# facebookresearch/SlowFast

Measured on NVIDIA H100. Metric: clips/sec (fwd+bwd) SlowFast-8x8-R50, higher is better.
Workload: dtype bf16x3-split operands, f32 accumulate/storage

## Files before the change

include/slowfast_b200.h:

```cpp
#ifndef SLOWFAST_B200_H_
#define SLOWFAST_B200_H_

#include <stdint.h>

#ifdef __cplusplus
extern "C" {
#endif

const char* sfb_last_error(void);
int sfb_abi_version(void);
const char* sfb_build_arch(void);

typedef struct sfb_conv_desc {
  const void* a_hi;
  const void* a_lo;
  int32_t n, d, h, w, c;
  int64_t c_pitch;
  const void* b_hi;
  const void* b_lo;
  int32_t cout;
  int32_t kt, kh, kw;
  int32_t dil_t, dil_h, dil_w;
  int32_t str_t, str_h, str_w;
  int32_t low_t, low_h, low_w;
// ... 44 lines not shown

int sfb_set_wgrad_direct(int32_t enabled);

int sfb_zero_f32_2d(float* ptr, int64_t rows, int64_t c, int64_t pitch, void* stream);

int sfb_add_f32_2d(float* dst, const float* src, int64_t rows, int32_t c, int64_t dst_pitch, int64_t src_pitch,
                   void* stream);

int sfb_split_planes(const float* x, int64_t rows, int32_t c, int64_t x_pitch, void* hi, void* lo,
                     int64_t o_pitch, void* stream);
int sfb_input_pack(const float* x, int32_t n, int32_t c, int32_t t, int32_t h, int32_t w, int32_t c_pad, void* hi,
                   void* lo, void* stream);
int sfb_filter_pack(const float* w, int32_t cout, int32_t cin, int32_t taps_total, const int32_t* tapmap,
                    int32_t ntaps, int32_t transpose, int32_t cols_pad, void* hi, void* lo, void* stream);
int sfb_filter_unpack_grad(const float* dwm, float* dw, int32_t cout, int32_t cin, int32_t taps, int32_t cin_pad,
                           int32_t accumulate, void* stream);

int sfb_bn_finalize(const float* partials, int32_t m_tiles, int32_t c, int64_t count, const float* gamma,
                    const float* beta, float* running_mean, float* running_var, float momentum, float eps,
                    int32_t training, float* scale, float* shift, float* save_mean, float* save_invstd,
                    int32_t affine_c, void* stream);

int32_t sfb_bn_split_stats_tiles(int64_t rows, int64_t rows_per_clip, int32_t splits, int32_t c);
int sfb_bn_split_stats(const float* y, int64_t y_pitch, int64_t rows, int32_t c, int32_t splits, int64_t rows_per_clip,
                       float* partials, void* stream);

typedef struct sfb_bn_apply_desc {
  const float* y; int64_t y_pitch; const float* scale; const float* shift;
  const float* y2; int64_t y2_pitch; const float* scale2; const float* shift2;
  const void* res_hi; const void* res_lo; int64_t res_pitch;
  void* out_hi; void* out_lo; int64_t out_pitch;
  int64_t rows; int32_t c; int32_t relu;
  int32_t splits; int64_t rows_per_clip;
} sfb_bn_apply_desc;
int sfb_bn_apply(const sfb_bn_apply_desc* d, void* stream);

typedef struct sfb_bn_bwd_desc {
  const float* dout; int64_t dout_pitch;
  const void* mask_hi; int64_t mask_pitch;
  const float* y; int64_t y_pitch;
  const float* mean; const float* invstd; const float* gamma;
  float* dgamma; float* dbeta; int32_t accumulate_param_grads;
  int32_t training;
  void* dy_hi; void* dy_lo; int64_t dy_pitch;
  float* dres; int64_t dres_pitch; int32_t dres_accumulate;
  float* partials;
  float* coef;
  int64_t rows; int32_t c;
  int32_t c_valid;
  const float* mask_scale; const float* mask_shift;
  int32_t splits; int64_t rows_per_clip;
} sfb_bn_bwd_desc;
int32_t sfb_bn_bwd_blocks(int64_t rows, int32_t c, int32_t splits, int64_t rows_per_clip);
int sfb_bn_bwd(const sfb_bn_bwd_desc* d, void* stream);

typedef struct sfb_pool_desc {
  const float* y; const float* scale; const float* shift;
  int32_t n, t, h, w, c, oh, ow, kh, kw, sh, sw, ph, pw;
  void* out_hi; void* out_lo; int64_t out_pitch;
  uint8_t* argmax;
  const float* dout; int64_t dout_pitch;
  float* dz;
  int32_t splits;
} sfb_pool_desc;
int sfb_bn_relu_maxpool_fwd(const sfb_pool_desc* d, void* stream);
int sfb_bn_relu_maxpool_bwd(const sfb_pool_desc* d, void* stream);



typedef struct sfb_pool3d_desc {
  const void* in_hi; const void* in_lo; int64_t in_pitch;
  void* out_hi; void* out_lo; int64_t out_pitch;
  uint8_t* argmax;
  int32_t n, t, h, w, c, ot, oh, ow;
  int32_t kt, kh, kw, st, sh, sw, pt, ph, pw;
  const float* dout; int64_t dout_pitch;
  float* din; int64_t din_pitch; int32_t din_accumulate;
} sfb_pool3d_desc;
int sfb_maxpool3d_fwd(const sfb_pool3d_desc* d, void* stream);
int sfb_maxpool3d_bwd(const sfb_pool3d_desc* d, void* stream);

int sfb_stem_input_fold(const float* x, int32_t n, int32_t cin, int32_t t, int32_t h, int32_t w, void* hi, void* lo,
                        void* stream);
int sfb_stem_filter_fold(const float* w, float* dw, int32_t cout, int32_t cin, int32_t kt, int32_t kh, int32_t kw,
// ... 261 lines not shown
```

slowfast_b200/csrc/elementwise.cu:

```cuda
#include <cstdint>
#include <cstring>
#include <cuda_bf16.h>

#include "../../include/slowfast_b200.h"
#include "planes.cuh"
#include "runtime.h"

namespace sfb {

static int ew_sms() {
  int sms = kGridSms;
  device_limits(&sms, nullptr);
  return sms;
}
static int ew_grid(int64_t items, int block) { return capped_grid(items, block, int64_t(ew_sms()) * 8); }
static int rowlane_grid(int64_t rows, int cg, int block) {
  const int lanes_c = cg < block ? cg : block;
  const int lanes_r = block / lanes_c;
  return capped_grid(rows, lanes_r * 4, int64_t(ew_sms()) * 8);
}

struct f32x8 {
  float4 a, b;
};
// ... 172 lines not shown
    for (int k = 0; k < 8; ++k) {
      sm[threadIdx.x * 16 + k] = s1[k];
      sm[threadIdx.x * 16 + 8 + k] = s2[k];
    }
    __syncthreads();
    if (lr == 0 && g < cg) {
      for (int q = 1; q < lanes_r; ++q) {
#pragma unroll
        for (int k = 0; k < 8; ++k) {
          s1[k] += sm[(q * lanes_c + lc) * 16 + k];
          s2[k] += sm[(q * lanes_c + lc) * 16 + 8 + k];
        }
      }
#pragma unroll
      for (int k = 0; k < 8; ++k) {
        const int64_t ch = int64_t(s) * p.c + g * 8 + k;
        p.partials[ch * p.blocks_per_split + col] = s1[k];
        p.partials[sq + ch * p.blocks_per_split + col] = s2[k];
      }
    }
    __syncthreads();
  }
}

struct BnApplyParams {
  const float* y; int64_t y_pitch;
  const float* scale; const float* shift;
  const float* y2; int64_t y2_pitch;
  const float* scale2; const float* shift2;
  const __nv_bfloat16* r_hi; const __nv_bfloat16* r_lo; int64_t r_pitch;
  __nv_bfloat16* o_hi; __nv_bfloat16* o_lo; int64_t o_pitch;
  int64_t rows; int c; int relu;
  int splits; int64_t rows_per_clip;
};
__device__ __forceinline__ int split_of_row(int64_t r, int64_t rows_per_clip, int splits) {
  return int((r / rows_per_clip) % splits);
}
struct RowLanes {
  int lanes_c, lanes_r, lc, lr;
  __device__ __forceinline__ RowLanes(int cg) {
    lanes_c = cg < int(blockDim.x) ? cg : int(blockDim.x);
    lanes_r = blockDim.x / lanes_c;
    lc = threadIdx.x % lanes_c;
    lr = threadIdx.x / lanes_c;
  }
};
__global__ void __launch_bounds__(256) bn_apply_kernel(const BnApplyParams p) {
  const int cg = p.c / 8;
  const RowLanes L(cg);
  if (L.lr >= L.lanes_r) return;
  for (int g = L.lc; g < cg; g += L.lanes_c) {
    const int c = g * 8;
    float sc[8], sh[8], sc2[8], sh2[8];
    load8(p.scale + c, sc);
    load8(p.shift + c, sh);
    if (p.y2) {
      load8(p.scale2 + c, sc2);
      load8(p.shift2 + c, sh2);
    }
    int cur = 0;
    for (int64_t r = int64_t(blockIdx.x) * L.lanes_r + L.lr; r < p.rows; r += int64_t(gridDim.x) * L.lanes_r) {
      if (p.splits > 1) {
        const int s = split_of_row(r, p.rows_per_clip, p.splits);
        if (s != cur) {
          cur = s;
          const int64_t o = int64_t(s) * p.c + c;
          load8(p.scale + o, sc);
          load8(p.shift + o, sh);
          if (p.y2) {
            load8(p.scale2 + o, sc2);
            load8(p.shift2 + o, sh2);
          }
        }
      }
      float v[8];
      load8(p.y + r * p.y_pitch + c, v);
#pragma unroll
      for (int j = 0; j < 8; ++j) v[j] = fmaf(v[j], sc[j], sh[j]);
      if (p.y2) {
        float w[8];
        load8(p.y2 + r * p.y2_pitch + c, w);
#pragma unroll
        for (int j = 0; j < 8; ++j) v[j] += fmaf(w[j], sc2[j], sh2[j]);
      }
      if (p.r_hi) {
        float w[8];
        load_planes8(p.r_hi + r * p.r_pitch + c, p.r_lo ? p.r_lo + r * p.r_pitch + c : nullptr, w);
#pragma unroll
        for (int j = 0; j < 8; ++j) v[j] += w[j];
      }
      if (p.relu) {
#pragma unroll
        for (int j = 0; j < 8; ++j) v[j] = fmaxf(v[j], 0.f);
      }
      store_split8(p.o_hi + r * p.o_pitch + c, p.o_lo ? p.o_lo + r * p.o_pitch + c : nullptr, v);
    }
  }
}

struct BnBwdReduceParams {
  const float* dout; int64_t dout_pitch;
  const __nv_bfloat16* mask; int64_t mask_pitch;
  const float* y; int64_t y_pitch;
  const float* mean; const float* invstd;
  int64_t rows; int c;
  float* partials;
  const float* mask_scale; const float* mask_shift;
  int splits; int64_t rows_per_clip; int blocks_per_clip;
};
__global__ void __launch_bounds__(256) bn_bwd_reduce_kernel(const BnBwdReduceParams p) {
  extern __shared__ float sm[];
  const int cg = p.c / 8;
  const int lanes_c = cg < int(blockDim.x) ? cg : int(blockDim.x);
  const int lanes_r = blockDim.x / lanes_c;
  const int lc = threadIdx.x % lanes_c;
  const int lr = threadIdx.x / lanes_c;
  int64_t r0, r1, coff = 0;
  if (p.splits > 1) {
    const int64_t clip = blockIdx.x / p.blocks_per_clip;
    const int64_t rpb = (p.rows_per_clip + p.blocks_per_clip - 1) / p.blocks_per_clip;
    r0 = clip * p.rows_per_clip + (blockIdx.x % p.blocks_per_clip) * rpb;
    r1 = min(r0 + rpb, (clip + 1) * p.rows_per_clip);
    coff = (clip % p.splits) * p.c;
  } else {
    const int64_t rows_per_block = (p.rows + gridDim.x - 1) / gridDim.x;
    r0 = blockIdx.x * rows_per_block;
    r1 = (r0 + rows_per_block < p.rows) ? r0 + rows_per_block : p.rows;
  }
  for (int g0 = 0; g0 < cg; g0 += lanes_c) {
    const int g = g0 + lc;
    float s1[8], s2[8];
#pragma unroll
    for (int j = 0; j < 8; ++j) s1[j] = s2[j] = 0.f;
    if (g < cg && lr < lanes_r) {
      const int c = g * 8;
      float mu[8], is[8], msc[8], msh[8];
      load8(p.mean + coff + c, mu);
      load8(p.invstd + coff + c, is);
      if (p.mask_scale) {
        load8(p.mask_scale + coff + c, msc);
        load8(p.mask_shift + coff + c, msh);
      }
      for (int64_t r = r0 + lr; r < r1; r += lanes_r) {
        float d[8], yv[8];
        load8(p.dout + r * p.dout_pitch + c, d);
        load8(p.y + r * p.y_pitch + c, yv);
        if (p.mask) {
          float m[8];
          load_planes8(p.mask + r * p.mask_pitch + c, nullptr, m);
#pragma unroll
          for (int j = 0; j < 8; ++j) d[j] = m[j] > 0.f ? d[j] : 0.f;
        } else if (p.mask_scale) {
#pragma unroll
          for (int j = 0; j < 8; ++j) d[j] = fmaf(yv[j], msc[j], msh[j]) > 0.f ? d[j] : 0.f;
        }
#pragma unroll
        for (int j = 0; j < 8; ++j) {
          s1[j] += d[j];
          s2[j] = fmaf(d[j], (yv[j] - mu[j]) * is[j], s2[j]);
        }
      }
    }
#pragma unroll
    for (int j = 0; j < 8; ++j) {
      sm[threadIdx.x * 16 + j] = s1[j];
      sm[threadIdx.x * 16 + 8 + j] = s2[j];
    }
    __syncthreads();
    if (lr == 0 && g < cg) {
      for (int k = 1; k < lanes_r; ++k) {
#pragma unroll
        for (int j = 0; j < 8; ++j) {
          s1[j] += sm[(k * lanes_c + lc) * 16 + j];
          s2[j] += sm[(k * lanes_c + lc) * 16 + 8 + j];
        }
      }
      float* out = p.partials + size_t(blockIdx.x) * 2 * p.c;
      store8(out + g * 8, s1);
      store8(out + p.c + g * 8, s2);
    }
    __syncthreads();
  }
}

__global__ void __launch_bounds__(64) bn_bwd_finalize_kernel(const float* __restrict__ partials, int nblocks, int c,
                                                             double count, const float* __restrict__ gamma,
                                                             const float* __restrict__ invstd,
                                                             float* __restrict__ dgamma, float* __restrict__ dbeta,
// ... 22 lines not shown
    __syncthreads();
    for (int o = 32; o > 0; o >>= 1) {
      if (threadIdx.x < o) {
        sm1[threadIdx.x] += sm1[threadIdx.x + o];
        sm2[threadIdx.x] += sm2[threadIdx.x + o];
      }
      __syncthreads();
    }
    if (threadIdx.x == 0) {
      s1 = sm1[0];
      s2 = sm2[0];
      t1 += s1;
      t2 += s2;
      const double a = double(gamma ? gamma[ch] : 1.f) * double(invstd[s * c + ch]);
      coef[s * c + ch] = float(a);
      coef[sc + s * c + ch] = training ? float(a * s1 / count) : 0.f;
      coef[2 * sc + s * c + ch] = training ? float(a * s2 / count) : 0.f;
    }
    __syncthreads();
  }
  if (threadIdx.x != 0) return;
  if (dgamma) dgamma[ch] = accumulate ? dgamma[ch] + float(t2) : float(t2);
  if (dbeta) dbeta[ch] = accumulate ? dbeta[ch] + float(t1) : float(t1);
}

struct BnBwdApplyParams {
  const float* dout; int64_t dout_pitch;
  const __nv_bfloat16* mask; int64_t mask_pitch;
  const float* y; int64_t y_pitch;
  const float* mean; const float* invstd; const float* coef;
  __nv_bfloat16* dy_hi; __nv_bfloat16* dy_lo; int64_t dy_pitch;
  float* dres; int64_t dres_pitch; int dres_accumulate;
  int64_t rows; int c;
  const float* mask_scale; const float* mask_shift;
  int splits; int64_t rows_per_clip;
};
struct BnBwdCoef {
  float mu[8], ca[8], cb[8], k1[8], msc[8], msh[8];
  __device__ __forceinline__ void load(const BnBwdApplyParams& p, int s, int c) {
    const int64_t o = int64_t(s) * p.c + c, sc = int64_t(p.splits > 1 ? p.splits : 1) * p.c;
    float is[8], cc[8];
    load8(p.mean + o, mu);
    load8(p.invstd + o, is);
    load8(p.coef + o, ca);
    load8(p.coef + sc + o, cb);
    load8(p.coef + 2 * sc + o, cc);
#pragma unroll
    for (int j = 0; j < 8; ++j) k1[j] = is[j] * cc[j];
    if (p.mask_scale) {
      load8(p.mask_scale + o, msc);
      load8(p.mask_shift + o, msh);
    }
  }
};
__global__ void __launch_bounds__(256) bn_bwd_apply_kernel(const BnBwdApplyParams p) {
  const int cg = p.c / 8;
  const RowLanes L(cg);
  if (L.lr >= L.lanes_r) return;
  for (int g = L.lc; g < cg; g += L.lanes_c) {
    const int c = g * 8;
    BnBwdCoef k;
    k.load(p, 0, c);
    float (&mu)[8] = k.mu, (&ca)[8] = k.ca, (&cb)[8] = k.cb, (&k1)[8] = k.k1, (&msc)[8] = k.msc, (&msh)[8] = k.msh;
    int cur = 0;
    for (int64_t r = int64_t(blockIdx.x) * L.lanes_r + L.lr; r < p.rows; r += int64_t(gridDim.x) * L.lanes_r) {
      if (p.splits > 1) {
        const int s = split_of_row(r, p.rows_per_clip, p.splits);
        if (s != cur) {
          cur = s;
          k.load(p, s, c);
        }
      }
      float d[8], yv[8];
      load8(p.dout + r * p.dout_pitch + c, d);
      load8(p.y + r * p.y_pitch + c, yv);
      if (p.mask) {
        float m[8];
        load_planes8(p.mask + r * p.mask_pitch + c, nullptr, m);
#pragma unroll
        for (int j = 0; j < 8; ++j) d[j] = m[j] > 0.f ? d[j] : 0.f;
      } else if (p.mask_scale) {
#pragma unroll
        for (int j = 0; j < 8; ++j) d[j] = fmaf(yv[j], msc[j], msh[j]) > 0.f ? d[j] : 0.f;
      }
      if (p.dres) {
        float* dr = p.dres + r * p.dres_pitch + c;
        if (p.dres_accumulate) {
          float o[8];
          load8(dr, o);
#pragma unroll
          for (int j = 0; j < 8; ++j) o[j] += d[j];
          store8(dr, o);
        } else {
          store8(dr, d);
        }
      }
      float gq[8];
#pragma unroll
      for (int j = 0; j < 8; ++j) gq[j] = ca[j] * d[j] - cb[j] - (yv[j] - mu[j]) * k1[j];
      store_split8(p.dy_hi + r * p.dy_pitch + c, p.dy_lo ? p.dy_lo + r * p.dy_pitch + c : nullptr, gq);
    }
  }
}

struct PoolParams {
  const float* y; const float* scale; const float* shift;
  int n, t, h, w, c; int oh, ow; int kh, kw, sh, sw, ph, pw;
  __nv_bfloat16* o_hi; __nv_bfloat16* o_lo; int64_t o_pitch;
  uint8_t* argmax;
  const float* dout; int64_t dout_pitch; float* dz;
  int splits;
};
__global__ void __launch_bounds__(256, 4) bn_relu_maxpool_fwd_kernel(const PoolParams p) {
  const int cg = p.c / 8;
  const int64_t items = int64_t(p.n) * p.t * p.oh * p.ow * cg;
  for (int64_t i = blockIdx.x * int64_t(blockDim.x) + threadIdx.x; i < items; i += int64_t(gridDim.x) * blockDim.x) {
    const int g = int(i % cg);
// ... 179 lines not shown
extern "C" int sfb_bn_split_stats(const float* y, int64_t y_pitch, int64_t rows, int32_t c, int32_t splits,
                                  int64_t rows_per_clip, float* partials, void* stream) {
  if (c % 8 || y_pitch % 4 || splits < 1 || rows_per_clip <= 0 || rows % rows_per_clip ||
      (rows / rows_per_clip) % splits) {
    set_error("sfb_bn_split_stats: c=%d (a multiple of 8), %lld rows in clips of %lld rows, %d splits", c,
              (long long)rows, (long long)rows_per_clip, splits);
    return -10;
  }
  SplitStatsParams p;
  p.y = y; p.y_pitch = y_pitch; p.rows_per_clip = rows_per_clip; p.chunk_rows = split_stats_chunk(c);
  p.c = c; p.splits = splits;
  p.chunks = int((rows_per_clip + p.chunk_rows - 1) / p.chunk_rows);
  p.blocks_per_split = sfb_bn_split_stats_tiles(rows, rows_per_clip, splits, c);
  p.partials = partials;
  const int64_t blocks = rows / rows_per_clip * p.chunks;
  if (blocks == 0) return 0;
  bn_split_stats_kernel<<<unsigned(blocks), 256, 256 * 16 * sizeof(float), (cudaStream_t)stream>>>(p);
  return launch_status("sfb_bn_split_stats");
}

extern "C" int sfb_bn_apply(const sfb_bn_apply_desc* d, void* stream) {
  if (d->c % 8) {
    set_error("sfb_bn_apply: c=%d must be a multiple of 8", d->c);
    return -10;
  }
  if (!split_geometry_ok("sfb_bn_apply", d->rows, d->splits, d->rows_per_clip)) return -10;
  BnApplyParams p;
  p.y = d->y; p.y_pitch = d->y_pitch; p.scale = d->scale; p.shift = d->shift;
  p.y2 = d->y2; p.y2_pitch = d->y2_pitch; p.scale2 = d->scale2; p.shift2 = d->shift2;
  p.r_hi = (const bf16*)d->res_hi; p.r_lo = (const bf16*)d->res_lo; p.r_pitch = d->res_pitch;
  p.o_hi = (bf16*)d->out_hi; p.o_lo = (bf16*)d->out_lo; p.o_pitch = d->out_pitch;
  p.rows = d->rows; p.c = d->c; p.relu = d->relu;
  p.splits = d->splits > 1 ? d->splits : 1; p.rows_per_clip = d->rows_per_clip;
  const int64_t items = d->rows * (d->c / 8);
  if (items == 0) return 0;
  bn_apply_kernel<<<rowlane_grid(d->rows, d->c / 8, 256), 256, 0, (cudaStream_t)stream>>>(p);
  return launch_status("sfb_bn_apply");
}

static int64_t bn_bwd_slabs(int64_t rows) {
  int64_t b = (rows + 15) / 16;
  const int64_t cap = int64_t(ew_sms()) * 4;
  if (b > cap) b = cap;
  if (b < 1) b = 1;
  return b;
}

static int32_t bn_bwd_blocks_per_clip(int64_t rows, int64_t rows_per_clip) {
  const int64_t clips = rows / rows_per_clip;
  int64_t per = (bn_bwd_slabs(rows) + clips - 1) / clips;
  const int64_t most = (rows_per_clip + 15) / 16;
  if (per > most) per = most;
  return int32_t(per < 1 ? 1 : per);
}

extern "C" int32_t sfb_bn_bwd_blocks(int64_t rows, int32_t c, int32_t splits, int64_t rows_per_clip) {
  (void)c;
  if (splits > 1 && rows_per_clip > 0)
    return int32_t(rows / rows_per_clip * bn_bwd_blocks_per_clip(rows, rows_per_clip));
  return int32_t(bn_bwd_slabs(rows));
}

extern "C" int sfb_bn_bwd(const sfb_bn_bwd_desc* d, void* stream_) {
  cudaStream_t stream = (cudaStream_t)stream_;
  if (d->c % 8) {
    set_error("sfb_bn_bwd: c=%d must be a multiple of 8", d->c);
    return -10;
  }
  if (!split_geometry_ok("sfb_bn_bwd", d->rows, d->splits, d->rows_per_clip)) return -10;
  const int splits = d->splits > 1 ? d->splits : 1;
  const int nblocks = sfb_bn_bwd_blocks(d->rows, d->c, splits, d->rows_per_clip);
  const int bpc = splits > 1 ? bn_bwd_blocks_per_clip(d->rows, d->rows_per_clip) : 1;
  BnBwdReduceParams r;
  r.dout = d->dout; r.dout_pitch = d->dout_pitch;
  r.mask = (const bf16*)d->mask_hi; r.mask_pitch = d->mask_pitch;
  r.mask_scale = d->mask_scale; r.mask_shift = d->mask_shift;
  r.y = d->y; r.y_pitch = d->y_pitch; r.mean = d->mean; r.invstd = d->invstd;
  r.rows = d->rows; r.c = d->c; r.partials = d->partials;
  r.splits = splits; r.rows_per_clip = d->rows_per_clip; r.blocks_per_clip = bpc;
  bn_bwd_reduce_kernel<<<nblocks, 256, 256 * 16 * sizeof(float), stream>>>(r);
  if (int rc = launch_status("sfb_bn_bwd(reduce)")) return rc;
  bn_bwd_finalize_kernel<<<d->c, 64, 0, stream>>>(d->partials, nblocks, d->c, double(d->rows / splits), d->gamma,
                                                                 d->invstd, d->dgamma, d->dbeta, d->accumulate_param_grads,
                                                                 d->training, d->coef,
                                                                 d->c_valid > 0 ? d->c_valid : d->c, splits, bpc);
  if (int rc = launch_status("sfb_bn_bwd(finalize)")) return rc;
  BnBwdApplyParams a;
  a.dout = d->dout; a.dout_pitch = d->dout_pitch;
  a.mask = (const bf16*)d->mask_hi; a.mask_pitch = d->mask_pitch;
  a.mask_scale = d->mask_scale; a.mask_shift = d->mask_shift;
  a.y = d->y; a.y_pitch = d->y_pitch; a.mean = d->mean; a.invstd = d->invstd; a.coef = d->coef;
  a.dy_hi = (bf16*)d->dy_hi; a.dy_lo = (bf16*)d->dy_lo; a.dy_pitch = d->dy_pitch;
  a.dres = d->dres; a.dres_pitch = d->dres_pitch; a.dres_accumulate = d->dres_accumulate;
  a.rows = d->rows; a.c = d->c;
  a.splits = splits; a.rows_per_clip = d->rows_per_clip;
  const int64_t items = d->rows * (d->c / 8);
  bn_bwd_apply_kernel<<<rowlane_grid(d->rows, d->c / 8, 256), 256, 0, stream>>>(a);
  return launch_status("sfb_bn_bwd(apply)");
}

extern "C" int sfb_bn_relu_maxpool_fwd(const sfb_pool_desc* d, void* stream) {
  if (d->c % 8 || d->kh * d->kw > 254) {
    set_error("sfb_bn_relu_maxpool_fwd: c=%d must be a multiple of 8 and the window < 255 taps", d->c);
    return -10;
  }
  PoolParams p;
  memset(&p, 0, sizeof(p));
  p.y = d->y; p.scale = d->scale; p.shift = d->shift;
  p.n = d->n; p.t = d->t; p.h = d->h; p.w = d->w; p.c = d->c; p.oh = d->oh; p.ow = d->ow;
  p.kh = d->kh; p.kw = d->kw; p.sh = d->sh; p.sw = d->sw; p.ph = d->ph; p.pw = d->pw;
  p.o_hi = (bf16*)d->out_hi; p.o_lo = (bf16*)d->out_lo; p.o_pitch = d->out_pitch; p.argmax = d->argmax;
  p.splits = d->splits > 1 ? d->splits : 1;
  if (d->n % p.splits) {
    set_error("sfb_bn_relu_maxpool_fwd: batch %d is not a multiple of %d splits", d->n, p.splits);
    return -10;
  }
  const int64_t items = int64_t(d->n) * d->t * d->oh * d->ow * (d->c / 8);
  bn_relu_maxpool_fwd_kernel<<<ew_grid(items, 256), 256, 0, (cudaStream_t)stream>>>(p);
  return launch_status("sfb_bn_relu_maxpool_fwd");
}

extern "C" int sfb_bn_relu_maxpool_bwd(const sfb_pool_desc* d, void* stream) {
  if (d->c % 8) {
// ... 178 lines not shown
```

slowfast_b200/engine.py:

```python
from __future__ import annotations

from typing import Dict, List, Optional, Sequence, Tuple

import torch
import torch.nn as nn

from . import ops
from .conv_plan import dgrad_out_view, dgrad_plan
from .ops import F32, F32View, Planes
from .subbn import is_sub_bn


class Storage:

    def __init__(self, n, t, h, w, pitch, nsplit, device, planes: bool = True):
        self.shape = (n, t, h, w, pitch)
        self.hi = torch.empty(self.shape if planes else (0, 0, 0, 0, pitch), dtype=torch.bfloat16, device=device)
        self.lo = torch.empty(self.shape, dtype=torch.bfloat16, device=device) if (nsplit == 3 and planes) else None
        self.grad: Optional[torch.Tensor] = None
        self.grad_written = False

    def ensure_grad(self) -> torch.Tensor:
        if self.grad is None:
            self.grad = torch.empty(self.shape, dtype=F32, device=self.hi.device)
# ... 196 lines not shown
        sbn = self._stats_bn(ctx.training)
        momentum = sbn.momentum if sbn.momentum is not None else 0.1
        ops.bn_finalize(stats, m_tiles, s * c, rows // s, bn.weight, bn.bias, sbn.running_mean, sbn.running_var,
                        momentum, sbn.eps, ctx.training, self.scale, self.shift, self.mean, self.invstd, affine_c=c)
        if self.bias is not None:
            ops.bn_conv_bias(self.bias, c, momentum, ctx.training, sbn.running_mean, self.scale, self.shift, self.mean,
                             splits=s)

    def fprop(self, x: Planes) -> torch.Tensor:
        ctx = self.ctx
        assert x.c == self.cin_pad, (self.name, x.c, self.cin_pad)
        geom = ops.fprop_geom(x, self.k, self.stride, self.pad)
        ot, oh, ow = geom.out
        f = ctx.buf((self.name, "f.hi"), (self.cout, self.taps * self.cin_pad), torch.bfloat16)
        flo = ctx.buf((self.name, "f.lo"), f.shape, torch.bfloat16) if ctx.nsplit == 3 else None
        fm = ops.FilterMat(f, flo, self.cout, self.taps, self.cin_pad)
        ops.filter_pack(self.conv.weight, fm)
        c, cp = self.cout, self.cout_pad
        y = ctx.buf((self.name, "y"), (x.n, ot, oh, ow, cp))
        strides = (ot * oh * ow * cp, oh * ow * cp, ow * cp, cp)
        m_tiles = ops.conv_stats_tiles(x, fm, geom, y, strides, nsplit=ctx.nsplit)
        self.splits = self.bn.num_splits if (self.sub and ctx.training) else 1
        self.rows_per_clip = ot * oh * ow
        stats = ctx.buf((self.name, "stats"), (2, c, m_tiles)) \
            if (ctx.training and self.bn is not None and self.splits == 1) else None
        ops.conv_igemm(x, fm, geom, y, strides, stats=stats, nsplit=ctx.nsplit)
        self.x, self.geom, self.y = x, geom, y
        if self.bn is None:
            return y
        self._bn_forward(y, stats, m_tiles, cp, zero=True)
        return y

    def bwd(self, dout: F32View, mask: Optional[Planes], x_act: Optional[Act], dres: Optional[F32View] = None,
            dres_accumulate: bool = False, mask_from_y: bool = False) -> None:
        ctx = self.ctx
        n, ot, oh, ow, c = self.y.shape
        dy = ctx.scratch_planes("dy", n, ot, oh, ow, c)
        partials, coef = self._bwd_scratch(n * ot * oh * ow, c)
        bn = self.bn
        ops.bn_bwd(dout, mask, ops.f32view(self.y), self.mean, self.invstd, bn.weight, ctx.grad_of(bn.weight),
                   ctx.grad_of(bn.bias), dy, partials, coef, training=ctx.training, dres=dres,
                   dres_accumulate=dres_accumulate, c_valid=self.cout,
                   mask_affine=(self.scale, self.shift) if mask_from_y else None, **self.split_kw)
        if self.bias is not None:
            rows = n * ot * oh * ow
            dyf = ctx.scratch("bias.dy", rows * c, F32).view(rows, c)
            ops.planes_to_f32(dy, ops.f32view(dyf))
            part = ctx.scratch("colsum.part", ops.colsum_blocks(rows) * self.cout, F32)
            ops.colsum(dyf, rows, self.cout, ctx.grad_of(self.bias), part, pitch=c)
        self.wgrad(dy)
        if x_act is not None:
            self.dgrad(dy, x_act)

    def _bwd_scratch(self, rows, c):
        nb = ops.bn_bwd_blocks(rows, c, self.splits, self.rows_per_clip)
        return (self.ctx.scratch("bnb.partials", nb * 2 * c, F32).view(nb, 2, c),
                self.ctx.scratch("bnb.coef", 3 * self.splits * c, F32).view(3, self.splits * c))

    def wgrad(self, dy: Planes) -> None:
        ctx = self.ctx
        gw = ctx.grad_of(self.conv.weight)
        if self.taps == 1 and self.cin_pad == self.cin and self.cout_pad == self.cout:
            ops.zero_f32(ops.f32view(gw.view(self.cout, self.cin)))
            ops.conv_wgrad(self.x, dy, self.geom, gw, nsplit=ctx.nsplit)
        else:
            dwm = ctx.scratch("dwm", self.cout_pad * self.taps * self.cin_pad, F32).view(self.cout_pad, -1)
            ops.zero_f32(ops.f32view(dwm))
            ops.conv_wgrad(self.x, dy, self.geom, dwm, nsplit=ctx.nsplit)
            ops.filter_unpack_grad(dwm, gw, self.cin_pad, accumulate=False)

    def dgrad(self, dy: Planes, x_act: Act) -> None:
        ctx = self.ctx
        _, t, h, w, pitch = x_act.s.shape
        plan = dgrad_plan((t, h, w), self.k, self.stride, self.pad)
        acc = x_act.s.grad_written
        g = x_act.s.ensure_grad()
# ... 226 lines not shown
```

slowfast_b200/lib.py:

```python
from __future__ import annotations

import ctypes as C
from pathlib import Path

from .build import lib_path


class NativeLibraryError(RuntimeError):
    pass


class ConvDesc(C.Structure):

    _fields_ = [
        ("a_hi", C.c_void_p), ("a_lo", C.c_void_p),
        ("n", C.c_int32), ("d", C.c_int32), ("h", C.c_int32), ("w", C.c_int32), ("c", C.c_int32),
        ("c_pitch", C.c_int64),
        ("b_hi", C.c_void_p), ("b_lo", C.c_void_p),
        ("cout", C.c_int32),
        ("kt", C.c_int32), ("kh", C.c_int32), ("kw", C.c_int32),
        ("dil_t", C.c_int32), ("dil_h", C.c_int32), ("dil_w", C.c_int32),
        ("str_t", C.c_int32), ("str_h", C.c_int32), ("str_w", C.c_int32),
        ("low_t", C.c_int32), ("low_h", C.c_int32), ("low_w", C.c_int32),
        ("out_t", C.c_int32), ("out_h", C.c_int32), ("out_w", C.c_int32),
# ... 7 lines not shown

class WgradDesc(C.Structure):

    _fields_ = [
        ("x_hi", C.c_void_p), ("x_lo", C.c_void_p),
        ("n", C.c_int32), ("d", C.c_int32), ("h", C.c_int32), ("w", C.c_int32), ("c", C.c_int32),
        ("c_pitch", C.c_int64),
        ("dy_hi", C.c_void_p), ("dy_lo", C.c_void_p),
        ("cout", C.c_int32), ("dy_pitch", C.c_int64),
        ("kt", C.c_int32), ("kh", C.c_int32), ("kw", C.c_int32),
        ("dil_t", C.c_int32), ("dil_h", C.c_int32), ("dil_w", C.c_int32),
        ("str_t", C.c_int32), ("str_h", C.c_int32), ("str_w", C.c_int32),
        ("low_t", C.c_int32), ("low_h", C.c_int32), ("low_w", C.c_int32),
        ("out_t", C.c_int32), ("out_h", C.c_int32), ("out_w", C.c_int32),
        ("dw", C.c_void_p),
        ("nsplit", C.c_int32),
    ]


class WgradPlan(C.Structure):

    _fields_ = [(name, C.c_int32) for name in ("direct", "transposed", "tile_rows", "bn", "ck", "tiles", "k_blocks",
                                               "slices", "ctas")]


class BnApplyDesc(C.Structure):
    _fields_ = [
        ("y", C.c_void_p), ("y_pitch", C.c_int64), ("scale", C.c_void_p), ("shift", C.c_void_p),
        ("y2", C.c_void_p), ("y2_pitch", C.c_int64), ("scale2", C.c_void_p), ("shift2", C.c_void_p),
        ("res_hi", C.c_void_p), ("res_lo", C.c_void_p), ("res_pitch", C.c_int64),
        ("out_hi", C.c_void_p), ("out_lo", C.c_void_p), ("out_pitch", C.c_int64),
        ("rows", C.c_int64), ("c", C.c_int32), ("relu", C.c_int32),
        ("splits", C.c_int32), ("rows_per_clip", C.c_int64),
    ]


class BnBwdDesc(C.Structure):
    _fields_ = [
        ("dout", C.c_void_p), ("dout_pitch", C.c_int64),
        ("mask_hi", C.c_void_p), ("mask_pitch", C.c_int64),
        ("y", C.c_void_p), ("y_pitch", C.c_int64),
        ("mean", C.c_void_p), ("invstd", C.c_void_p), ("gamma", C.c_void_p),
        ("dgamma", C.c_void_p), ("dbeta", C.c_void_p), ("accumulate_param_grads", C.c_int32),
        ("training", C.c_int32),
        ("dy_hi", C.c_void_p), ("dy_lo", C.c_void_p), ("dy_pitch", C.c_int64),
        ("dres", C.c_void_p), ("dres_pitch", C.c_int64), ("dres_accumulate", C.c_int32),
        ("partials", C.c_void_p), ("coef", C.c_void_p),
        ("rows", C.c_int64), ("c", C.c_int32), ("c_valid", C.c_int32),
        ("mask_scale", C.c_void_p), ("mask_shift", C.c_void_p),
        ("splits", C.c_int32), ("rows_per_clip", C.c_int64),
    ]


class OptChunk(C.Structure):

    _fields_ = [("param", C.c_void_p), ("offset", C.c_int64), ("count", C.c_int32), ("group", C.c_int32)]


class MomentumChunk(C.Structure):

    _fields_ = [("key", C.c_void_p), ("query", C.c_void_p), ("count", C.c_int64)]


class PoolDesc(C.Structure):
    _fields_ = [
        ("y", C.c_void_p), ("scale", C.c_void_p), ("shift", C.c_void_p),
        ("n", C.c_int32), ("t", C.c_int32), ("h", C.c_int32), ("w", C.c_int32), ("c", C.c_int32),
        ("oh", C.c_int32), ("ow", C.c_int32), ("kh", C.c_int32), ("kw", C.c_int32),
        ("sh", C.c_int32), ("sw", C.c_int32), ("ph", C.c_int32), ("pw", C.c_int32),
        ("out_hi", C.c_void_p), ("out_lo", C.c_void_p), ("out_pitch", C.c_int64),
        ("argmax", C.c_void_p),
        ("dout", C.c_void_p), ("dout_pitch", C.c_int64),
        ("dz", C.c_void_p),
        ("splits", C.c_int32),
    ]


class DwPoolDesc(C.Structure):
    _fields_ = [
        ("src", C.c_void_p), ("src_pitch", C.c_int64), ("src_c0", C.c_int32), ("bias", C.c_void_p),
        ("w", C.c_void_p), ("out", C.c_void_p),
        ("b", C.c_int32), ("heads", C.c_int32), ("hd", C.c_int32), ("t", C.c_int32), ("h", C.c_int32),
        ("w_", C.c_int32), ("ot", C.c_int32), ("oh", C.c_int32), ("ow", C.c_int32),
# ... 295 lines not shown
```

slowfast_b200/nets/resnet.py:

```python
from __future__ import annotations

from typing import List, Optional

import torch
import torch.nn as nn

from .. import ops
from ..config import nsplit_of
from ..engine import Act, ConvBN, Ctx, ModelFunction, Namespace, StemConvBN, bump_num_batches_tracked
from ..ops import F32, Planes
from ..subbn import is_sub_bn, norm_factory, num_splits_of

STAGE_DEPTH = {18: (2, 2, 2, 2), 50: (3, 4, 6, 3), 101: (3, 4, 23, 3)}

TEMPORAL_KERNELS = {
    "2d": [[[1]], [[1]], [[1]], [[1]], [[1]]],
    "c2d": [[[1]], [[1]], [[1]], [[1]], [[1]]],
    "slow_c2d": [[[1]], [[1]], [[1]], [[1]], [[1]]],
    "i3d": [[[5]], [[3]], [[3, 1]], [[3, 1]], [[1, 3]]],
    "slow_i3d": [[[5]], [[3]], [[3, 1]], [[3, 1]], [[1, 3]]],
    "slow": [[[1]], [[1]], [[1]], [[3]], [[3]]],
    "slowfast": [[[1], [5]], [[1], [3]], [[1], [3]], [[3], [3]], [[3], [3]]],
}
POOL1 = {"2d": [[1, 1, 1]], "c2d": [[2, 1, 1]], "slow_c2d": [[1, 1, 1]], "i3d": [[2, 1, 1]], "slow_i3d": [[1, 1, 1]],
# ... 52 lines not shown
        self.relu = nn.ReLU(True)
        self._n = name
        self._ctx = ctx
        self._dim_inner, self._dim_out = dim_inner, dim_out
        object.__setattr__(self, "_units", None)

    def units(self):
        if self._units is None:
            b2, n, ctx = self.branch2, self._n, self._ctx
            u = {"a": ConvBN(n + ".a", b2.a, b2.a_bn, ctx), "b": ConvBN(n + ".b", b2.b, b2.b_bn, ctx),
                 "c": ConvBN(n + ".c", b2.c, b2.c_bn, ctx)}
            if hasattr(self, "branch1"):
                u["s"] = ConvBN(n + ".branch1", self.branch1, self.branch1_bn, ctx)
            object.__setattr__(self, "_units", u)
        return self._units

    def out_dims(self, t, h, w):
        u = self.units()
        return u["b"].out_dims(*u["a"].out_dims(t, h, w))

    def bns(self):
        return [u.bn for u in self.units().values()]

    def run_forward(self, x: Act, out: Act) -> None:
        ctx, u, nm = self._ctx, self.units(), self._n
        n, t, h, w = x.dims
        ya = u["a"].fprop(x.planes)
        xa = Act(ctx.storage((nm, "xa"), *ya.shape))
        ops.bn_apply(ops.f32view(ya), u["a"].scale, u["a"].shift, xa.planes, relu=True, **u["a"].split_kw)
        yb = u["b"].fprop(xa.planes)
        xb = Act(ctx.storage((nm, "xb"), *yb.shape))
        ops.bn_apply(ops.f32view(yb), u["b"].scale, u["b"].shift, xb.planes, relu=True, **u["b"].split_kw)
        yc = u["c"].fprop(xb.planes)
        if "s" in u:
            ys = u["s"].fprop(x.planes)
            ops.bn_apply(ops.f32view(yc), u["c"].scale, u["c"].shift, out.planes, relu=True, y2=ops.f32view(ys),
                         scale2=u["s"].scale, shift2=u["s"].shift, **u["c"].split_kw)
        else:
            ops.bn_apply(ops.f32view(yc), u["c"].scale, u["c"].shift, out.planes, relu=True, res=x.planes,
                         **u["c"].split_kw)
        object.__setattr__(self, "_saved", (x, xa, xb, out))

    def run_backward(self) -> None:
        u = self.units()
        x, xa, xb, out = self._saved
        dout = out.grad_view()
        if "s" in u:
            u["s"].bwd(dout, out.planes, x)
            u["c"].bwd(dout, out.planes, xb)
        else:
            acc = x.s.grad_written
            u["c"].bwd(dout, out.planes, xb, dres=x.grad_view(), dres_accumulate=acc)
            x.s.grad_written = True
        u["b"].bwd(xb.grad_view(), xb.planes, xa)
        u["a"].bwd(xa.grad_view(), xa.planes, x)


NONLOCAL_INSTANTIATIONS = ("softmax", "dot_product")


class NonlocalModule(Namespace):

    def __init__(self, name, dim, dim_inner, pool_size, instantiation, group, ctx: Ctx, eps=1e-5, mmt=0.1,
                 norm=nn.BatchNorm3d):
        super().__init__()
        if instantiation not in NONLOCAL_INSTANTIATIONS:
            raise NotImplementedError(f"Unknown norm type {instantiation}")
        self.conv_theta = nn.Conv3d(dim, dim_inner, kernel_size=1, stride=1, padding=0)
        self.conv_phi = nn.Conv3d(dim, dim_inner, kernel_size=1, stride=1, padding=0)
        self.conv_g = nn.Conv3d(dim, dim_inner, kernel_size=1, stride=1, padding=0)
        self.conv_out = nn.Conv3d(dim_inner, dim, kernel_size=1, stride=1, padding=0)
        self.conv_out.zero_init = False
        self.bn = norm(num_features=dim, eps=eps, momentum=mmt)
        self.bn.transform_final_bn = True
        self.use_pool = pool_size is not None and any(s > 1 for s in pool_size)
        self.pool_size = tuple(int(s) for s in pool_size) if pool_size is not None else None
        if self.use_pool:
            self.pool = nn.MaxPool3d(kernel_size=list(pool_size), stride=list(pool_size), padding=[0, 0, 0])
        assert dim % 8 == 0 and dim_inner % 8 == 0, "Non-local widths must be multiples of 8"
        self.instantiation = instantiation
        self.dim, self.dim_inner, self.group = dim, dim_inner, int(group)
        self._n = name
        self._ctx = ctx
        object.__setattr__(self, "_units", None)

    def units(self):
        if self._units is None:
            n, ctx = self._n, self._ctx
# ... 499 lines not shown
                    else:
                        full = None
                        out = Act(ctx.storage((f"s{i}", p, bi), n, t, h, w, cout))
                    stage.run_block_forward(p, bi, x, out, (f"s{i}", p, bi))
                    x = full if full is not None else out
                outs.append(x)
            slow, fast = outs
            if i < 5:
                cs = stage.blocks(0)[-1]._dim_out
                self._fuse_forward(i, fast, slow.slice(cs, slow.c - cs))
            trace.append((slow, fast, cs))
        self._trace = trace
        if ctx.training:
            bump_num_batches_tracked(self._train_bns())
        out = self._head_forward([slow, fast])
        return out

    def _fuse_forward(self, i: int, fast: Act, out: Act) -> None:
        unit = self._engine_units()[f"fuse{i}"]
        y = unit.fprop(fast.planes)
        ops.bn_apply(ops.f32view(y), unit.scale, unit.shift, out.planes, relu=True, **unit.split_kw)
        self.__dict__.setdefault("_fuse_saved", {})[i] = (fast, out)

    def _engine_backward(self, dlogits: torch.Tensor):
        ctx = self.ctx
        params = [p for p in self.parameters()]
        ctx.begin_backward(params)
        u = self._engine_units()
        self._head_backward(dlogits)
        for i in range(5, 1, -1):
            stage: StageModule = getattr(self, f"s{i}")
            if i < 5:
                fast, out = self._fuse_saved[i]
                u[f"fuse{i}"].bwd(out.grad_view(), out.planes, fast)
            for p in (0, 1):
                for bi in reversed(range(stage.num_blocks[p])):
                    stage.run_block_backward(p, bi)
        fast, out = self._fuse_saved[1]
        u["fuse1"].bwd(out.grad_view(), out.planes, fast)
        self._stem_backward(0, u["stem0"])
        self._stem_backward(1, u["stem1"])
        return [ctx.grad_of(p) for p in params]
```

slowfast_b200/ops.py:

```python
from __future__ import annotations

import ctypes as C
import math
from dataclasses import dataclass
from typing import Optional, Sequence, Tuple

import torch

from . import lib as L

BF16 = torch.bfloat16
F32 = torch.float32

_launches = 0


def launches() -> int:
    return _launches


def _count(n: int = 1) -> None:
    global _launches
    _launches += n

# ... 247 lines not shown

def conv_wgrad(x: Planes, dy: Planes, geom: ConvGeom, dwm: torch.Tensor, nsplit: int = 3) -> None:
    lib = L.load()
    d = _wgrad_desc(x, dy, geom, dwm, nsplit)
    L.check(lib.sfb_conv_wgrad(C.byref(d), _stream()), "sfb_conv_wgrad")
    _count()


def bn_finalize(partials: Optional[torch.Tensor], m_tiles: int, c: int, count: int, gamma, beta, running_mean,
                running_var, momentum: float, eps: float, training: bool, scale, shift, save_mean, save_invstd,
                affine_c: int = 0):
    lib = L.load()
    L.check(lib.sfb_bn_finalize(_ptr(partials), m_tiles, c, count, _ptr(gamma), _ptr(beta), _ptr(running_mean),
                                _ptr(running_var), momentum, eps, 1 if training else 0, scale.data_ptr(),
                                shift.data_ptr(), _ptr(save_mean), _ptr(save_invstd), affine_c, _stream()),
            "sfb_bn_finalize")
    _count()


def bn_split_stats_tiles(rows: int, rows_per_clip: int, splits: int, c: int) -> int:
    return L.load().sfb_bn_split_stats_tiles(rows, rows_per_clip, splits, c)


def bn_split_stats(y: F32View, splits: int, rows_per_clip: int, partials: torch.Tensor) -> None:
    lib = L.load()
    tiles = bn_split_stats_tiles(y.rows, rows_per_clip, splits, y.c)
    assert partials.dtype == F32 and partials.numel() >= 2 * splits * y.c * tiles
    L.check(lib.sfb_bn_split_stats(y.ptr(), y.pitch, y.rows, y.c, splits, rows_per_clip, partials.data_ptr(),
                                   _stream()), "sfb_bn_split_stats")
    _count()


def bn_apply(y: F32View, scale, shift, out: Planes, relu: bool, y2: Optional[F32View] = None, scale2=None,
             shift2=None, res: Optional[Planes] = None, splits: int = 1, rows_per_clip: int = 0) -> None:
    lib = L.load()
    d = L.BnApplyDesc()
    d.splits, d.rows_per_clip = splits, rows_per_clip
    d.y, d.y_pitch, d.scale, d.shift = y.ptr(), y.pitch, scale.data_ptr(), shift.data_ptr()
    if y2 is not None:
        d.y2, d.y2_pitch, d.scale2, d.shift2 = y2.ptr(), y2.pitch, scale2.data_ptr(), shift2.data_ptr()
    if res is not None:
        assert res.c == out.c and res.rows == out.rows
        d.res_hi, d.res_lo, d.res_pitch = res.hi_ptr(), res.lo_ptr(), res.pitch
    d.out_hi, d.out_lo, d.out_pitch = out.hi_ptr(), out.lo_ptr(), out.pitch
    d.rows, d.c, d.relu = out.rows, out.c, 1 if relu else 0
    assert y.rows == out.rows and y.c == out.c
    L.check(lib.sfb_bn_apply(C.byref(d), _stream()), "sfb_bn_apply")
    _count()


def bn_bwd_blocks(rows: int, c: int, splits: int = 1, rows_per_clip: int = 0) -> int:
    return L.load().sfb_bn_bwd_blocks(rows, c, splits, rows_per_clip)


def bn_bwd_scratch(rows: int, c: int, device, splits: int = 1, rows_per_clip: int = 0):
    nb = bn_bwd_blocks(rows, c, splits, rows_per_clip)
    return (torch.empty((nb, 2, c), dtype=F32, device=device), torch.empty((3, splits * c), dtype=F32, device=device))


def bn_bwd(dout: F32View, mask: Optional[Planes], y: F32View, mean, invstd, gamma, dgamma, dbeta, dy: Planes,
           partials, coef, training: bool = True, accumulate_param_grads: bool = False,
           dres: Optional[F32View] = None, dres_accumulate: bool = False, c_valid: int = 0,
           mask_affine=None, splits: int = 1, rows_per_clip: int = 0) -> None:
    lib = L.load()
    d = L.BnBwdDesc()
    d.c_valid = c_valid
    d.splits, d.rows_per_clip = splits, rows_per_clip
    if mask_affine is not None:
        assert mask is None
        d.mask_scale, d.mask_shift = mask_affine[0].data_ptr(), mask_affine[1].data_ptr()
    d.dout, d.dout_pitch = dout.ptr(), dout.pitch
    if mask is not None:
        d.mask_hi, d.mask_pitch = mask.hi_ptr(), mask.pitch
    d.y, d.y_pitch = y.ptr(), y.pitch
    d.mean, d.invstd, d.gamma = mean.data_ptr(), invstd.data_ptr(), _ptr(gamma)
    d.dgamma, d.dbeta = _ptr(dgamma), _ptr(dbeta)
    d.accumulate_param_grads = 1 if accumulate_param_grads else 0
    d.training = 1 if training else 0
    d.dy_hi, d.dy_lo, d.dy_pitch = dy.hi_ptr(), dy.lo_ptr(), dy.pitch
    if dres is not None:
        d.dres, d.dres_pitch, d.dres_accumulate = dres.ptr(), dres.pitch, 1 if dres_accumulate else 0
    d.partials, d.coef = partials.data_ptr(), coef.data_ptr()
    d.rows, d.c = dy.rows, dy.c
    assert dout.rows == dy.rows and y.rows == dy.rows
    L.check(lib.sfb_bn_bwd(C.byref(d), _stream()), "sfb_bn_bwd")
    _count(3)


def _pool_desc(n, t, h, w, c, oh, ow, k, s, p):
    d = L.PoolDesc()
    d.n, d.t, d.h, d.w, d.c, d.oh, d.ow = n, t, h, w, c, oh, ow
    d.kh, d.kw = k
    d.sh, d.sw = s
    d.ph, d.pw = p
    return d


def bn_relu_maxpool_fwd(y: torch.Tensor, scale, shift, out: Planes, argmax: torch.Tensor, k, s, p,
                        splits: int = 1) -> None:
    lib = L.load()
    n, t, h, w, c = y.shape
    d = _pool_desc(n, t, h, w, c, out.h, out.w, k, s, p)
    d.splits = splits
# ... 876 lines not shown
```

Before: 195.2.

## Use packed relu bitmasks and recomputed masks in BN backward instead of bf16 planes

The forward bn_apply for the block output now also writes a 1-bit-per-channel relu mask. Backward BN for the c and shortcut units reads this packed byte instead of the bf16 hi plane of the output. For the a, b and fuse BNs, the relu mask is recomputed in backward from y with scale/shift, rounded to bf16 to match the stored activation, instead of loading the activation plane. This cuts backward memory traffic but adds a small extra write in forward and a bitmask buffer per block.

Measured after the change: 200.9 (median of 6 runs). +2.9%, better.

```diff
diff --git a/include/slowfast_b200.h b/include/slowfast_b200.h
--- a/include/slowfast_b200.h
+++ b/include/slowfast_b200.h
@@ -100,6 +100,7 @@
   void* out_hi; void* out_lo; int64_t out_pitch;
   int64_t rows; int32_t c; int32_t relu;
   int32_t splits; int64_t rows_per_clip;
+  uint8_t* mask_bits;
 } sfb_bn_apply_desc;
 int sfb_bn_apply(const sfb_bn_apply_desc* d, void* stream);
 
@@ -118,6 +119,8 @@
   int32_t c_valid;
   const float* mask_scale; const float* mask_shift;
   int32_t splits; int64_t rows_per_clip;
+  int32_t mask_round;
+  const uint8_t* mask_bits;
 } sfb_bn_bwd_desc;
 int32_t sfb_bn_bwd_blocks(int64_t rows, int32_t c, int32_t splits, int64_t rows_per_clip);
 int sfb_bn_bwd(const sfb_bn_bwd_desc* d, void* stream);
diff --git a/slowfast_b200/csrc/elementwise.cu b/slowfast_b200/csrc/elementwise.cu
--- a/slowfast_b200/csrc/elementwise.cu
+++ b/slowfast_b200/csrc/elementwise.cu
@@ -228,6 +228,7 @@
   __nv_bfloat16* o_hi; __nv_bfloat16* o_lo; int64_t o_pitch;
   int64_t rows; int c; int relu;
   int splits; int64_t rows_per_clip;
+  uint8_t* mask_bits;
 };
 __device__ __forceinline__ int split_of_row(int64_t r, int64_t rows_per_clip, int splits) {
   return int((r / rows_per_clip) % splits);
@@ -290,6 +291,12 @@
         for (int j = 0; j < 8; ++j) v[j] = fmaxf(v[j], 0.f);
       }
       store_split8(p.o_hi + r * p.o_pitch + c, p.o_lo ? p.o_lo + r * p.o_pitch + c : nullptr, v);
+      if (p.mask_bits) {
+        unsigned b = 0;
+#pragma unroll
+        for (int j = 0; j < 8; ++j) b |= unsigned(__bfloat162float(__float2bfloat16_rn(v[j])) > 0.f) << j;
+        p.mask_bits[r * cg + g] = uint8_t(b);
+      }
     }
   }
 }
@@ -302,8 +309,31 @@
   int64_t rows; int c;
   float* partials;
   const float* mask_scale; const float* mask_shift;
+  int mask_round;
+  const uint8_t* mask_bits;
   int splits; int64_t rows_per_clip; int blocks_per_clip;
 };
+template <class P>
+__device__ __forceinline__ void relu_mask8(const P& p, int64_t r, int c, const float (&yv)[8], const float (&msc)[8],
+                                           const float (&msh)[8], float (&d)[8]) {
+  if (p.mask_bits) {
+    const unsigned b = p.mask_bits[r * (p.c / 8) + c / 8];
+#pragma unroll
+    for (int j = 0; j < 8; ++j) d[j] = (b >> j) & 1u ? d[j] : 0.f;
+  } else if (p.mask) {
+    float m[8];
+    load_planes8(p.mask + r * p.mask_pitch + c, nullptr, m);
+#pragma unroll
+    for (int j = 0; j < 8; ++j) d[j] = m[j] > 0.f ? d[j] : 0.f;
+  } else if (p.mask_scale) {
+#pragma unroll
+    for (int j = 0; j < 8; ++j) {
+      const float z = fmaf(yv[j], msc[j], msh[j]);
+      d[j] = (p.mask_round ? __bfloat162float(__float2bfloat16_rn(z)) : z) > 0.f ? d[j] : 0.f;
+    }
+  }
+}
+
 __global__ void __launch_bounds__(256) bn_bwd_reduce_kernel(const BnBwdReduceParams p) {
   extern __shared__ float sm[];
   const int cg = p.c / 8;
@@ -341,15 +371,7 @@
         float d[8], yv[8];
         load8(p.dout + r * p.dout_pitch + c, d);
         load8(p.y + r * p.y_pitch + c, yv);
-        if (p.mask) {
-          float m[8];
-          load_planes8(p.mask + r * p.mask_pitch + c, nullptr, m);
-#pragma unroll
-          for (int j = 0; j < 8; ++j) d[j] = m[j] > 0.f ? d[j] : 0.f;
-        } else if (p.mask_scale) {
-#pragma unroll
-          for (int j = 0; j < 8; ++j) d[j] = fmaf(yv[j], msc[j], msh[j]) > 0.f ? d[j] : 0.f;
-        }
+        relu_mask8(p, r, c, yv, msc, msh, d);
 #pragma unroll
         for (int j = 0; j < 8; ++j) {
           s1[j] += d[j];
@@ -438,7 +460,8 @@
   __nv_bfloat16* dy_hi; __nv_bfloat16* dy_lo; int64_t dy_pitch;
   float* dres; int64_t dres_pitch; int dres_accumulate;
   int64_t rows; int c;
-  const float* mask_scale; const float* mask_shift;
+  const float* mask_scale; const float* mask_shift; int mask_round;
+  const uint8_t* mask_bits;
   int splits; int64_t rows_per_clip;
 };
 struct BnBwdCoef {
@@ -480,15 +503,7 @@
       float d[8], yv[8];
       load8(p.dout + r * p.dout_pitch + c, d);
       load8(p.y + r * p.y_pitch + c, yv);
-      if (p.mask) {
-        float m[8];
-        load_planes8(p.mask + r * p.mask_pitch + c, nullptr, m);
-#pragma unroll
-        for (int j = 0; j < 8; ++j) d[j] = m[j] > 0.f ? d[j] : 0.f;
-      } else if (p.mask_scale) {
-#pragma unroll
-        for (int j = 0; j < 8; ++j) d[j] = fmaf(yv[j], msc[j], msh[j]) > 0.f ? d[j] : 0.f;
-      }
+      relu_mask8(p, r, c, yv, msc, msh, d);
       if (p.dres) {
         float* dr = p.dres + r * p.dres_pitch + c;
         if (p.dres_accumulate) {
@@ -734,6 +749,7 @@
   p.o_hi = (bf16*)d->out_hi; p.o_lo = (bf16*)d->out_lo; p.o_pitch = d->out_pitch;
   p.rows = d->rows; p.c = d->c; p.relu = d->relu;
   p.splits = d->splits > 1 ? d->splits : 1; p.rows_per_clip = d->rows_per_clip;
+  p.mask_bits = d->mask_bits;
   const int64_t items = d->rows * (d->c / 8);
   if (items == 0) return 0;
   bn_apply_kernel<<<rowlane_grid(d->rows, d->c / 8, 256), 256, 0, (cudaStream_t)stream>>>(p);
@@ -776,7 +792,8 @@
   BnBwdReduceParams r;
   r.dout = d->dout; r.dout_pitch = d->dout_pitch;
   r.mask = (const bf16*)d->mask_hi; r.mask_pitch = d->mask_pitch;
-  r.mask_scale = d->mask_scale; r.mask_shift = d->mask_shift;
+  r.mask_scale = d->mask_scale; r.mask_shift = d->mask_shift; r.mask_round = d->mask_round;
+  r.mask_bits = d->mask_bits;
   r.y = d->y; r.y_pitch = d->y_pitch; r.mean = d->mean; r.invstd = d->invstd;
   r.rows = d->rows; r.c = d->c; r.partials = d->partials;
   r.splits = splits; r.rows_per_clip = d->rows_per_clip; r.blocks_per_clip = bpc;
@@ -790,7 +807,8 @@
   BnBwdApplyParams a;
   a.dout = d->dout; a.dout_pitch = d->dout_pitch;
   a.mask = (const bf16*)d->mask_hi; a.mask_pitch = d->mask_pitch;
-  a.mask_scale = d->mask_scale; a.mask_shift = d->mask_shift;
+  a.mask_scale = d->mask_scale; a.mask_shift = d->mask_shift; a.mask_round = d->mask_round;
+  a.mask_bits = d->mask_bits;
   a.y = d->y; a.y_pitch = d->y_pitch; a.mean = d->mean; a.invstd = d->invstd; a.coef = d->coef;
   a.dy_hi = (bf16*)d->dy_hi; a.dy_lo = (bf16*)d->dy_lo; a.dy_pitch = d->dy_pitch;
   a.dres = d->dres; a.dres_pitch = d->dres_pitch; a.dres_accumulate = d->dres_accumulate;
diff --git a/slowfast_b200/engine.py b/slowfast_b200/engine.py
--- a/slowfast_b200/engine.py
+++ b/slowfast_b200/engine.py
@@ -252,7 +252,8 @@
         return y
 
     def bwd(self, dout: F32View, mask: Optional[Planes], x_act: Optional[Act], dres: Optional[F32View] = None,
-            dres_accumulate: bool = False, mask_from_y: bool = False) -> None:
+            dres_accumulate: bool = False, mask_from_y: bool = False, mask_round: bool = False,
+            mask_bits: Optional[torch.Tensor] = None) -> None:
         ctx = self.ctx
         n, ot, oh, ow, c = self.y.shape
         dy = ctx.scratch_planes("dy", n, ot, oh, ow, c)
@@ -261,7 +262,8 @@
         ops.bn_bwd(dout, mask, ops.f32view(self.y), self.mean, self.invstd, bn.weight, ctx.grad_of(bn.weight),
                    ctx.grad_of(bn.bias), dy, partials, coef, training=ctx.training, dres=dres,
                    dres_accumulate=dres_accumulate, c_valid=self.cout,
-                   mask_affine=(self.scale, self.shift) if mask_from_y else None, **self.split_kw)
+                   mask_affine=(self.scale, self.shift) if mask_from_y else None, mask_round=mask_round,
+                   mask_bits=mask_bits, **self.split_kw)
         if self.bias is not None:
             rows = n * ot * oh * ow
             dyf = ctx.scratch("bias.dy", rows * c, F32).view(rows, c)
diff --git a/slowfast_b200/lib.py b/slowfast_b200/lib.py
--- a/slowfast_b200/lib.py
+++ b/slowfast_b200/lib.py
@@ -63,6 +63,7 @@
         ("out_hi", C.c_void_p), ("out_lo", C.c_void_p), ("out_pitch", C.c_int64),
         ("rows", C.c_int64), ("c", C.c_int32), ("relu", C.c_int32),
         ("splits", C.c_int32), ("rows_per_clip", C.c_int64),
+        ("mask_bits", C.c_void_p),
     ]
 
 
@@ -80,6 +81,7 @@
         ("rows", C.c_int64), ("c", C.c_int32), ("c_valid", C.c_int32),
         ("mask_scale", C.c_void_p), ("mask_shift", C.c_void_p),
         ("splits", C.c_int32), ("rows_per_clip", C.c_int64),
+        ("mask_round", C.c_int32), ("mask_bits", C.c_void_p),
     ]
 
 
diff --git a/slowfast_b200/nets/resnet.py b/slowfast_b200/nets/resnet.py
--- a/slowfast_b200/nets/resnet.py
+++ b/slowfast_b200/nets/resnet.py
@@ -108,28 +108,31 @@
         xb = Act(ctx.storage((nm, "xb"), *yb.shape))
         ops.bn_apply(ops.f32view(yb), u["b"].scale, u["b"].shift, xb.planes, relu=True, **u["b"].split_kw)
         yc = u["c"].fprop(xb.planes)
+        bits = ctx.buf((nm, "mask_bits"), (out.planes.rows, out.c // 8), torch.uint8)
         if "s" in u:
             ys = u["s"].fprop(x.planes)
             ops.bn_apply(ops.f32view(yc), u["c"].scale, u["c"].shift, out.planes, relu=True, y2=ops.f32view(ys),
-                         scale2=u["s"].scale, shift2=u["s"].shift, **u["c"].split_kw)
+                         scale2=u["s"].scale, shift2=u["s"].shift, mask_bits=bits, **u["c"].split_kw)
         else:
             ops.bn_apply(ops.f32view(yc), u["c"].scale, u["c"].shift, out.planes, relu=True, res=x.planes,
-                         **u["c"].split_kw)
+                         mask_bits=bits, **u["c"].split_kw)
         object.__setattr__(self, "_saved", (x, xa, xb, out))
+        object.__setattr__(self, "_mask_bits", bits)
 
     def run_backward(self) -> None:
         u = self.units()
         x, xa, xb, out = self._saved
+        bits = self._mask_bits
         dout = out.grad_view()
         if "s" in u:
-            u["s"].bwd(dout, out.planes, x)
-            u["c"].bwd(dout, out.planes, xb)
+            u["s"].bwd(dout, None, x, mask_bits=bits)
+            u["c"].bwd(dout, None, xb, mask_bits=bits)
         else:
             acc = x.s.grad_written
-            u["c"].bwd(dout, out.planes, xb, dres=x.grad_view(), dres_accumulate=acc)
+            u["c"].bwd(dout, None, xb, dres=x.grad_view(), dres_accumulate=acc, mask_bits=bits)
             x.s.grad_written = True
-        u["b"].bwd(xb.grad_view(), xb.planes, xa)
-        u["a"].bwd(xa.grad_view(), xa.planes, x)
+        u["b"].bwd(xb.grad_view(), None, xa, mask_from_y=True, mask_round=True)
+        u["a"].bwd(xa.grad_view(), None, x, mask_from_y=True, mask_round=True)
 
 
 NONLOCAL_INSTANTIATIONS = ("softmax", "dot_product")
@@ -695,12 +698,12 @@
             stage: StageModule = getattr(self, f"s{i}")
             if i < 5:
                 fast, out = self._fuse_saved[i]
-                u[f"fuse{i}"].bwd(out.grad_view(), out.planes, fast)
+                u[f"fuse{i}"].bwd(out.grad_view(), None, fast, mask_from_y=True, mask_round=True)
             for p in (0, 1):
                 for bi in reversed(range(stage.num_blocks[p])):
                     stage.run_block_backward(p, bi)
         fast, out = self._fuse_saved[1]
-        u["fuse1"].bwd(out.grad_view(), out.planes, fast)
+        u["fuse1"].bwd(out.grad_view(), None, fast, mask_from_y=True, mask_round=True)
         self._stem_backward(0, u["stem0"])
         self._stem_backward(1, u["stem1"])
         return [ctx.grad_of(p) for p in params]
diff --git a/slowfast_b200/ops.py b/slowfast_b200/ops.py
--- a/slowfast_b200/ops.py
+++ b/slowfast_b200/ops.py
@@ -303,10 +303,15 @@
 
 
 def bn_apply(y: F32View, scale, shift, out: Planes, relu: bool, y2: Optional[F32View] = None, scale2=None,
-             shift2=None, res: Optional[Planes] = None, splits: int = 1, rows_per_clip: int = 0) -> None:
+             shift2=None, res: Optional[Planes] = None, splits: int = 1, rows_per_clip: int = 0,
+             mask_bits: Optional[torch.Tensor] = None) -> None:
     lib = L.load()
     d = L.BnApplyDesc()
     d.splits, d.rows_per_clip = splits, rows_per_clip
+    if mask_bits is not None:
+        assert mask_bits.dtype == torch.uint8 and mask_bits.is_contiguous() and \
+            mask_bits.numel() == out.rows * (out.c // 8)
+        d.mask_bits = mask_bits.data_ptr()
     d.y, d.y_pitch, d.scale, d.shift = y.ptr(), y.pitch, scale.data_ptr(), shift.data_ptr()
     if y2 is not None:
         d.y2, d.y2_pitch, d.scale2, d.shift2 = y2.ptr(), y2.pitch, scale2.data_ptr(), shift2.data_ptr()
@@ -332,14 +337,20 @@
 def bn_bwd(dout: F32View, mask: Optional[Planes], y: F32View, mean, invstd, gamma, dgamma, dbeta, dy: Planes,
            partials, coef, training: bool = True, accumulate_param_grads: bool = False,
            dres: Optional[F32View] = None, dres_accumulate: bool = False, c_valid: int = 0,
-           mask_affine=None, splits: int = 1, rows_per_clip: int = 0) -> None:
+           mask_affine=None, splits: int = 1, rows_per_clip: int = 0, mask_round: bool = False,
+           mask_bits: Optional[torch.Tensor] = None) -> None:
     lib = L.load()
     d = L.BnBwdDesc()
     d.c_valid = c_valid
     d.splits, d.rows_per_clip = splits, rows_per_clip
+    assert (mask is not None) + (mask_affine is not None) + (mask_bits is not None) <= 1
     if mask_affine is not None:
-        assert mask is None
         d.mask_scale, d.mask_shift = mask_affine[0].data_ptr(), mask_affine[1].data_ptr()
+        d.mask_round = 1 if mask_round else 0
+    if mask_bits is not None:
+        assert mask_bits.dtype == torch.uint8 and mask_bits.is_contiguous() and \
+            mask_bits.numel() == dy.rows * (dy.c // 8)
+        d.mask_bits = mask_bits.data_ptr()
     d.dout, d.dout_pitch = dout.ptr(), dout.pitch
     if mask is not None:
         d.mask_hi, d.mask_pitch = mask.hi_ptr(), mask.pitch
```
